# jiwoon-ahn/irn

Hardware: AMD Instinct MI355X
Metric: images/sec for CAM+random-walk label gen, VOC12 512^2 (random-walk label generation stage) (higher is better)
Workload: dtype f32

## Files before the change

irn_amd/csrc/affinity.hip:

```cpp
#include "path_unroll.hpp"

namespace irn {

namespace {

__device__ __forceinline__ float pow_beta(float a, float beta, int beta_int) {
    double b = (double)a;
    if (beta_int > 0) {
        double r = 1.0;
        int e = beta_int;
        while (e) {
            if (e & 1) r *= b;
            b *= b;
            e >>= 1;
        }
        return (float)r;
    }
    return (float)pow(b, (double)beta);
}

template <bool POW>
__global__ __launch_bounds__(256) void affinity_kernel(const AffJob *__restrict__ jobs,
                                                       const int *__restrict__ dir_start8,
                                                       const int *__restrict__ cell_off8, int n_dirs,
                                                       int radius, float beta, int beta_int) {
    extern __shared__ float tile[];
    const AffJob J = jobs[blockIdx.y];
    const int tiles_x = (J.sw + AFF_TW - 1) / AFF_TW;
    const int tiles_y = (J.sh + AFF_TH - 1) / AFF_TH;
    if ((int)blockIdx.x >= tiles_x * tiles_y) return;
    const int halo = radius - 1;
    const int LW = AFF_TW + 2 * halo;
    const int LH = AFF_TH + halo;
    const int ty0 = ((int)blockIdx.x / tiles_x) * AFF_TH;
    const int tx0 = ((int)blockIdx.x % tiles_x) * AFF_TW;

    for (int i = threadIdx.x; i < LH * LW; i += 256) {
        const int ly = i / LW, lx = i - ly * LW;
        const int gy = J.oy + ty0 + ly;
        const int gx = J.ox + tx0 + lx - halo;
        float v = 1.0f;
        if (gy < J.gh && gx >= 0 && gx < J.gw) v = J.edge[(long)gy * J.gw + gx];
        tile[i] = v;
    }
    __syncthreads();

    const int ly = threadIdx.x / AFF_TW, lx = threadIdx.x % AFF_TW;
    const int sy = ty0 + ly, sx = tx0 + lx;
    const bool valid = sy < J.sh && sx < J.sw;
    const int base = ly * LW + lx + halo;
    float *out = J.out + (long)sy * J.sw + sx;

    const float *tb = tile + base;
    for (int d = 0; d < n_dirs; ++d) {
        const int k0 = dir_start8[d], k1 = dir_start8[d + 1];
        float m0 = -INFINITY, m1 = -INFINITY;
        for (int k = k0; k < k1; k += 8) {
            const int4 oa = *reinterpret_cast<const int4 *>(cell_off8 + k);
            const int4 ob = *reinterpret_cast<const int4 *>(cell_off8 + k + 4);
            const float a0 = tb[oa.x], a1 = tb[oa.y], a2 = tb[oa.z], a3 = tb[oa.w];
            const float b0 = tb[ob.x], b1 = tb[ob.y], b2 = tb[ob.z], b3 = tb[ob.w];
            m0 = max3(max3(m0, a0, a1), a2, a3);
            m1 = max3(max3(m1, b0, b1), b2, b3);
        }
        const float m = max3(m0, m1, m1);
        float a = 1.0f - m;
        if (POW) a = pow_beta(a, beta, beta_int);
        if (valid) out[(long)d * J.plane_stride] = a;
    }
}

template <int R>
__global__ __launch_bounds__(256) void affinity_unrolled_kernel(const AffJob *__restrict__ jobs, int beta_int) {
    constexpr int HALO = R - 1, LW = AFF_TW + 2 * HALO, LH = AFF_TH + HALO, ND = kPaths<R>.n_dirs;
    __shared__ float tile[LH * LW];
    const AffJob J = jobs[blockIdx.y];
    const int tiles_x = (J.sw + AFF_TW - 1) / AFF_TW;
    const int tiles_y = (J.sh + AFF_TH - 1) / AFF_TH;
    if ((int)blockIdx.x >= tiles_x * tiles_y) return;
    const int ty0 = ((int)blockIdx.x / tiles_x) * AFF_TH;
    const int tx0 = ((int)blockIdx.x % tiles_x) * AFF_TW;
    for (int i = threadIdx.x; i < LH * LW; i += 256) {
        const int ly = i / LW, lx = i - ly * LW;
        const int gy = J.oy + ty0 + ly;
        const int gx = J.ox + tx0 + lx - HALO;
        float v = 1.0f;
        if (gy < J.gh && gx >= 0 && gx < J.gw) v = J.edge[(long)gy * J.gw + gx];
        tile[i] = v;
    }
    __syncthreads();
    const int ly = threadIdx.x / AFF_TW, lx = threadIdx.x % AFF_TW;
    const int sy = ty0 + ly, sx = tx0 + lx;
    const bool valid = sy < J.sh && sx < J.sw;
    const float *tb = tile + ly * LW + lx;
    float *out = J.out + (long)sy * J.sw + sx;
    static_for<ND>([&](auto id) __attribute__((always_inline)) {
        constexpr int d = decltype(id)::value;
        double b = (double)(1.0f - path_max<R, d>(tb)), r = 1.0;
        for (int e = beta_int; e; e >>= 1) {
            if (e & 1) r *= b;
            b *= b;
        }
        if (valid) *out = (float)r;
        out += J.plane_stride;
    });
}

__global__ __launch_bounds__(256) void affinity_backward_kernel(const AffJob *__restrict__ jobs,
                                                                const float *const *__restrict__ grad_aff,
                                                                float *const *__restrict__ grad_edge,
                                                                const int *__restrict__ dir_start,
                                                                const int *__restrict__ cell_dy,
                                                                const int *__restrict__ cell_dx, int n_dirs, int radius) {
    extern __shared__ float tile[];
    const AffJob J = jobs[blockIdx.y];
    const int tiles_x = (J.sw + AFF_TW - 1) / AFF_TW;
    const int tiles_y = (J.sh + AFF_TH - 1) / AFF_TH;
    if ((int)blockIdx.x >= tiles_x * tiles_y) return;
    const int halo = radius - 1;
    const int LW = AFF_TW + 2 * halo;
    const int LH = AFF_TH + halo;
    float *gtile = tile + LH * LW;
    const int ty0 = ((int)blockIdx.x / tiles_x) * AFF_TH;
    const int tx0 = ((int)blockIdx.x % tiles_x) * AFF_TW;
    for (int i = threadIdx.x; i < LH * LW; i += 256) {
        const int ly = i / LW, lx = i - ly * LW;
        const int gy = J.oy + ty0 + ly;
        const int gx = J.ox + tx0 + lx - halo;
        float v = 1.0f;
        if (gy < J.gh && gx >= 0 && gx < J.gw) v = J.edge[(long)gy * J.gw + gx];
        tile[i] = v;
        gtile[i] = 0.f;
    }
    __syncthreads();
    const int ly = threadIdx.x / AFF_TW, lx = threadIdx.x % AFF_TW;
    const int sy = ty0 + ly, sx = tx0 + lx;
    const bool valid = sy < J.sh && sx < J.sw;
    const int base = ly * LW + lx + halo;
    const float *ga = grad_aff[blockIdx.y] + (long)sy * J.sw + sx;
    if (valid) {
        for (int d = 0; d < n_dirs; ++d) {
            const int k0 = dir_start[d], k1 = dir_start[d + 1];
            float m = -INFINITY;
            int arg = 0;
            for (int k = k0; k < k1; ++k) {
                const int off = cell_dy[k] * LW + cell_dx[k];
                const float v = tile[base + off];
                if (v > m) {
                    m = v;
                    arg = off;
                }
            }
            atomicAdd(&gtile[base + arg], -ga[(long)d * J.plane_stride]);
        }
    }
    __syncthreads();
    float *ge = grad_edge[blockIdx.y];
    for (int i = threadIdx.x; i < LH * LW; i += 256) {
        const float g = gtile[i];
        if (g == 0.f) continue;
        const int py = i / LW, px = i - py * LW;
        const int gy = J.oy + ty0 + py;
        const int gx = J.ox + tx0 + px - halo;
        if (gy < J.gh && gx >= 0 && gx < J.gw) unsafeAtomicAdd(ge + (long)gy * J.gw + gx, g);
    }
}

}

int launch_affinity(const AffJob *jobs_dev, int n_jobs, int max_sh, int max_sw, const DeviceTable &tab,
                    bool with_pow, float beta, hipStream_t stream) {
    const int tiles = cdiv(max_sh, AFF_TH) * cdiv(max_sw, AFF_TW);
    const int halo = tab.radius - 1;
    const size_t lds = sizeof(float) * (AFF_TH + halo) * (AFF_TW + 2 * halo);
    dim3 grid(tiles, n_jobs);
    int beta_int = 0;
    if (with_pow && beta == (float)(int)beta && beta >= 1.0f && beta <= 64.0f) beta_int = (int)beta;
    if (with_pow && beta_int > 0 && tab.order == 1 && tab.radius == 10)
        hipLaunchKernelGGL(affinity_unrolled_kernel<10>, grid, dim3(256), 0, stream, jobs_dev, beta_int);
    else if (with_pow && beta_int > 0 && tab.order == 1 && tab.radius == 5)
        hipLaunchKernelGGL(affinity_unrolled_kernel<5>, grid, dim3(256), 0, stream, jobs_dev, beta_int);
    else if (with_pow)
        hipLaunchKernelGGL(affinity_kernel<true>, grid, dim3(256), lds, stream, jobs_dev, tab.dir_start8,
                           tab.cell_off8, tab.n_dirs, tab.radius, beta, beta_int);
    else
        hipLaunchKernelGGL(affinity_kernel<false>, grid, dim3(256), lds, stream, jobs_dev, tab.dir_start8,
                           tab.cell_off8, tab.n_dirs, tab.radius, beta, beta_int);
    IRN_LAUNCH_CHECK("affinity_kernel");
    return IRN_OK;
}

}

using namespace irn;

extern "C" int irn_version(void) { return 100; }

extern "C" const char *irn_last_error(void) { return last_error_slot().c_str(); }

extern "C" int irn_path_count(int radius, int *n_dirs, int *n_cells) {
    if (radius < 2 || radius > IRN_MAX_RADIUS || !n_dirs || !n_cells)
        return fail(IRN_ERR_ARG, "irn_path_count: radius must be in [2,%d]", IRN_MAX_RADIUS);
    PathTable t = build_path_table(radius, 0);
    *n_dirs = t.n_dirs();
    *n_cells = t.n_cells();
    return IRN_OK;
}

extern "C" int irn_path_table(int radius, int order, int32_t *dst_dydx, int32_t *path_start,
                              int32_t *cells_dydx) {
    if (radius < 2 || radius > IRN_MAX_RADIUS || (order != 0 && order != 1) || !dst_dydx || !path_start ||
        !cells_dydx)
        return fail(IRN_ERR_ARG, "irn_path_table: bad argument");
    PathTable t = build_path_table(radius, order);
    for (int i = 0; i < t.n_dirs(); ++i) {
        dst_dydx[2 * i] = t.dy[i];
        dst_dydx[2 * i + 1] = t.dx[i];
    }
    for (int i = 0; i <= t.n_dirs(); ++i) path_start[i] = t.start[i];
    for (int i = 0; i < t.n_cells(); ++i) {
        cells_dydx[2 * i] = t.cy[i];
        cells_dydx[2 * i + 1] = t.cx[i];
    }
    return IRN_OK;
}

extern "C" int irn_edge_to_affinity(const float *edge_dev, int batch, int hp, int wp, int radius,
                                    float *aff_dev, void *stream_) {
    hipStream_t stream = (hipStream_t)stream_;
    if (!edge_dev || !aff_dev || batch < 1 || radius < 2 || radius > IRN_MAX_RADIUS)
        return fail(IRN_ERR_ARG, "irn_edge_to_affinity: bad argument");
    const int rf = radius - 1;
    const int sh = hp - rf, sw = wp - 2 * rf;
    if (sh < 1 || sw < 1)
        return fail(IRN_ERR_ARG, "irn_edge_to_affinity: grid %dx%d too small for radius %d", hp, wp, radius);
    const DeviceTable *tab = nullptr;
    int rc = get_device_table(radius, 0, &tab);
    if (rc) return rc;
    std::vector<AffJob> jobs(batch);
    const long ns = (long)sh * sw;
    for (int b = 0; b < batch; ++b) {
        AffJob &j = jobs[b];
        j.edge = edge_dev + (long)b * hp * wp;
        j.out = aff_dev + (long)b * tab->n_dirs * ns;
        j.gh = hp; j.gw = wp; j.oy = 0; j.ox = rf; j.sh = sh; j.sw = sw;
        j.plane_stride = ns;
    }
    AffJob *jobs_dev = nullptr;
    rc = scratch_upload(jobs.data(), sizeof(AffJob) * batch, (void **)&jobs_dev, stream);
    if (rc) return rc;
    rc = launch_affinity(jobs_dev, batch, sh, sw, *tab, false, 0.f, stream);
    if (rc) return rc;
    return scratch_release(stream);
}

extern "C" int irn_edge_to_affinity_backward(const float *edge_dev, const float *grad_aff_dev, int batch, int hp, int wp,
                                             int radius, float *grad_edge_dev, void *stream_) {
    hipStream_t stream = (hipStream_t)stream_;
    if (!edge_dev || !grad_aff_dev || !grad_edge_dev || batch < 1 || radius < 2 || radius > IRN_MAX_RADIUS)
        return fail(IRN_ERR_ARG, "irn_edge_to_affinity_backward: bad argument");
    const int rf = radius - 1;
    const int sh = hp - rf, sw = wp - 2 * rf;
    if (sh < 1 || sw < 1)
        return fail(IRN_ERR_ARG, "irn_edge_to_affinity_backward: grid %dx%d too small for radius %d", hp, wp, radius);
    const DeviceTable *tab = nullptr;
    int rc = get_device_table(radius, 0, &tab);
    if (rc) return rc;
    const long ns = (long)sh * sw;
    std::vector<char> host(sizeof(AffJob) * batch + 2 * sizeof(void *) * batch);
    AffJob *jobs = (AffJob *)host.data();
    const float **gas = (const float **)(host.data() + sizeof(AffJob) * batch);
    float **ges = (float **)(host.data() + sizeof(AffJob) * batch + sizeof(void *) * batch);
    for (int b = 0; b < batch; ++b) {
        AffJob &j = jobs[b];
        j.edge = edge_dev + (long)b * hp * wp;
        j.out = nullptr;
        j.gh = hp; j.gw = wp; j.oy = 0; j.ox = rf; j.sh = sh; j.sw = sw;
        j.plane_stride = ns;
        gas[b] = grad_aff_dev + (long)b * tab->n_dirs * ns;
        ges[b] = grad_edge_dev + (long)b * hp * wp;
    }
    char *dev = nullptr;
    rc = scratch_upload(host.data(), host.size(), (void **)&dev, stream);
    if (rc) return rc;
    IRN_HIP_TRY(hipMemsetAsync(grad_edge_dev, 0, sizeof(float) * (size_t)batch * hp * wp, stream));
    const int tiles = cdiv(sh, AFF_TH) * cdiv(sw, AFF_TW);
    const size_t lds = 2 * sizeof(float) * (AFF_TH + rf) * (AFF_TW + 2 * rf);
    hipLaunchKernelGGL(affinity_backward_kernel, dim3(tiles, batch), dim3(256), lds, stream, (const AffJob *)dev,
                       (const float *const *)(dev + sizeof(AffJob) * batch),
                       (float *const *)(dev + sizeof(AffJob) * batch + sizeof(void *) * batch), tab->dir_start, tab->cell_dy,
                       tab->cell_dx, tab->n_dirs, radius);
    IRN_LAUNCH_CHECK("affinity_backward_kernel");
    return scratch_release(stream);
}

namespace {
__global__ __launch_bounds__(256) void pair_disp_kernel(const float *__restrict__ disp, float *__restrict__ out, int hp,
                                                        int wp, int rf, int n_dirs, const int *__restrict__ dir_dy,
                                                        const int *__restrict__ dir_dx) {
    const int ch = hp - rf, cw = wp - 2 * rf;
    const int s = blockIdx.x * 256 + threadIdx.x;
    if (s >= ch * cw) return;
    const int y = s / cw, x = s - y * cw;
    const float *plane = disp + (size_t)blockIdx.y * hp * wp;
    float *o = out + (size_t)blockIdx.y * n_dirs * ch * cw + s;
    const float src = plane[y * wp + rf + x];
    for (int d = 0; d < n_dirs; ++d)
        o[(size_t)d * ch * cw] = src - plane[(y + dir_dy[d]) * wp + rf + x + dir_dx[d]];
}

__global__ __launch_bounds__(256) void pair_disp_backward_kernel(const float *__restrict__ gout, float *__restrict__ gdisp,
                                                                 int hp, int wp, int rf, int n_dirs,
                                                                 const int *__restrict__ dir_dy, const int *__restrict__ dir_dx) {
    const int ch = hp - rf, cw = wp - 2 * rf;
    const int p = blockIdx.x * 256 + threadIdx.x;
    if (p >= hp * wp) return;
    const int Y = p / wp, X = p - Y * wp;
    const float *g = gout + (size_t)blockIdx.y * n_dirs * ch * cw;
    const int xs = X - rf;
    float acc = 0.f;
    if (Y < ch && xs >= 0 && xs < cw)
        for (int d = 0; d < n_dirs; ++d) acc += g[(size_t)d * ch * cw + Y * cw + xs];
    for (int d = 0; d < n_dirs; ++d) {
        const int yy = Y - dir_dy[d], xx = xs - dir_dx[d];
        if (yy >= 0 && yy < ch && xx >= 0 && xx < cw) acc -= g[(size_t)d * ch * cw + yy * cw + xx];
    }
    gdisp[(size_t)blockIdx.y * hp * wp + p] = acc;
}

int pair_disp_args(const char *who, const void *a, const void *b, int batch, int channels, int hp, int wp, int radius,
                   const DeviceTable **tab) {
    if (!a || !b || batch < 1 || channels < 1 || radius < 2 || radius > IRN_MAX_RADIUS)
        return fail(IRN_ERR_ARG, "%s: bad argument", who);
    if (hp - (radius - 1) < 1 || wp - 2 * (radius - 1) < 1)
        return fail(IRN_ERR_ARG, "%s: grid %dx%d too small for radius %d", who, hp, wp, radius);
    if ((long)batch * channels > 65535) return fail(IRN_ERR_ARG, "%s: batch * channels must be <= 65535", who);
    return get_device_table(radius, 0, tab);
}
}

extern "C" int irn_pair_displacement(const float *disp_dev, int batch, int channels, int hp, int wp, int radius,
                                     float *out_dev, void *stream) {
    const DeviceTable *tab = nullptr;
    if (int rc = pair_disp_args("irn_pair_displacement", disp_dev, out_dev, batch, channels, hp, wp, radius, &tab)) return rc;
    const int rf = radius - 1;
    hipLaunchKernelGGL(pair_disp_kernel, dim3(cdiv((hp - rf) * (wp - 2 * rf), 256), batch * channels), dim3(256), 0,
                       (hipStream_t)stream, disp_dev, out_dev, hp, wp, rf, tab->n_dirs, tab->dir_dy, tab->dir_dx);
    IRN_LAUNCH_CHECK("pair_disp_kernel");
    return IRN_OK;
}

extern "C" int irn_pair_displacement_backward(const float *grad_out_dev, int batch, int channels, int hp, int wp,
                                              int radius, float *grad_disp_dev, void *stream) {
    const DeviceTable *tab = nullptr;
    if (int rc = pair_disp_args("irn_pair_displacement_backward", grad_out_dev, grad_disp_dev, batch, channels, hp, wp,
                                radius, &tab))
        return rc;
    hipLaunchKernelGGL(pair_disp_backward_kernel, dim3(cdiv(hp * wp, 256), batch * channels), dim3(256), 0,
                       (hipStream_t)stream, grad_out_dev, grad_disp_dev, hp, wp, radius - 1, tab->n_dirs, tab->dir_dy,
                       tab->dir_dx);
    IRN_LAUNCH_CHECK("pair_disp_backward_kernel");
    return IRN_OK;
}
```

irn_amd/csrc/kernels.hpp:

```cpp
#pragma once
#include "common.hpp"

namespace irn {

struct DeviceTable {
    int radius = 0, order = 0, n_dirs = 0, n_cells = 0;
    int *dir_dy = nullptr, *dir_dx = nullptr;
    int *dir_start = nullptr;
    int *cell_dy = nullptr, *cell_dx = nullptr;
    int *cell_off8 = nullptr;
    int *dir_start8 = nullptr;
    int *plane_tab = nullptr;
    PathTable host;
};

int get_device_table(int radius, int order, const DeviceTable **out);

int scratch_upload(const void *host, size_t bytes, void **dev_out, hipStream_t stream);
int scratch_release(hipStream_t stream);

constexpr int kAffTileH = 8, kAffTileW = 32;

struct AffJob {
    const float *edge;
    float *out;
    int gh, gw;
    int oy, ox;
    int sh, sw;
    long plane_stride;
};

int launch_affinity(const AffJob *jobs_dev, int n_jobs, int max_sh, int max_sw, const DeviceTable &tab,
                    bool with_pow, float beta, hipStream_t stream);

}
```

irn_amd/csrc/path_unroll.hpp:

```cpp
#pragma once
#include <utility>

#include "kernels.hpp"

namespace irn {

constexpr int AFF_TH = kAffTileH;
constexpr int AFF_TW = kAffTileW;

__device__ __forceinline__ float max3(float a, float b, float c) {
    float r;
    asm("v_max3_f32 %0, %1, %2, %3" : "=v"(r) : "v"(a), "v"(b), "v"(c));
    return r;
}

template <int R>
struct Paths {
    static constexpr int kMaxDirs = 2 * R * R, kMaxCells = 32 * R * R;
    int n_dirs = 0, n_cells = 0;
    signed char dy[kMaxDirs] = {}, dx[kMaxDirs] = {};
    short start[kMaxDirs + 1] = {};
    signed char cy[kMaxCells] = {}, cx[kMaxCells] = {};
    constexpr void add(int y, int x) {
        dy[n_dirs] = (signed char)y;
        dx[n_dirs] = (signed char)x;
        const int lsq = y * y + x * x;
        const int x_lo = x < 0 ? x : 0, x_hi = x < 0 ? 0 : x;
        for (int py = 0; py <= y; ++py)
            for (int px = x_lo; px <= x_hi; ++px) {
                const int cross = y * px - x * py;
                if (cross * cross < lsq) {
                    cy[n_cells] = (signed char)py;
                    cx[n_cells] = (signed char)px;
                    ++n_cells;
                }
            }
        start[++n_dirs] = (short)n_cells;
    }
    constexpr Paths() {
        for (int x = 1; x < R; ++x) add(0, x);
        for (int y = 1; y < R; ++y)
            for (int x = -R + 1; x < R; ++x)
                if (x * x + y * y < R * R) add(y, x);
    }
};
template <int R>
inline constexpr Paths<R> kPaths{};

template <int... Is, typename F>
__device__ __forceinline__ void static_for_impl(std::integer_sequence<int, Is...>, F &&f) {
    (f(std::integral_constant<int, Is>{}), ...);
}
template <int N, typename F>
__device__ __forceinline__ void static_for(F &&f) {
    static_for_impl(std::make_integer_sequence<int, N>{}, f);
}

template <int R, int D>
__device__ __forceinline__ float path_max(const float *tb) {
    constexpr int LW = AFF_TW + 2 * (R - 1), HALO = R - 1;
    constexpr int k0 = kPaths<R>.start[D], n = kPaths<R>.start[D + 1] - k0;
    constexpr auto off = [](int k) constexpr { return kPaths<R>.cy[k] * LW + kPaths<R>.cx[k] + HALO; };
    float m = tb[off(k0)];
    static_for<(n - 1) / 2>([&](auto ik) __attribute__((always_inline)) {
        constexpr int k = k0 + 1 + 2 * decltype(ik)::value;
        m = max3(m, tb[off(k)], tb[off(k + 1)]);
    });
    if constexpr ((n - 1) % 2 == 1) {
        const float v = tb[off(k0 + n - 1)];
        m = max3(m, v, v);
    }
    return m;
}

}
```

irn_amd/csrc/walk.hip:

```cpp
#include <algorithm>
#include <cmath>
#include <mutex>

#include "walk_ctx.hpp"

namespace irn {


namespace {


__global__ __launch_bounds__(256) void zero_pad_kernel(const WalkImg *__restrict__ imgs, int n_dirs) {
    const WalkImg I = imgs[blockIdx.y];
    const int d = blockIdx.x;
    if (d >= n_dirs) return;
    float *plane = I.wts + (long)d * I.plane_stride;
    for (int i = threadIdx.x; i < I.front_pad; i += 256) plane[-1 - i] = 0.f;
    const long n = (long)I.h * I.w;
    const long end = I.plane_stride - I.front_pad;
    for (long i = n + threadIdx.x; i < end; i += 256) plane[i] = 0.f;
}

__global__ __launch_bounds__(256) void degree_kernel(const WalkImg *__restrict__ imgs,
                                                     const int *__restrict__ dir_dy,
// ... 454 lines not shown
    } else {
        return fail(IRN_ERR_ARG, "irn_walk_set_option: unknown option '%s'", name);
    }
    ctx->n = 0;
    return IRN_OK;
}

extern "C" int irn_walk_enable_timing(irn_walk_ctx *ctx, int enable) {
    if (!ctx) return fail(IRN_ERR_ARG, "null ctx");
    ctx->timing = enable ? 1 : 0;
    return IRN_OK;
}

extern "C" int irn_walk_last_sweep_ms(irn_walk_ctx *ctx, float *ms, int *n_launches) {
    if (!ctx || !ms || !n_launches) return fail(IRN_ERR_ARG, "null argument");
    if (ctx->ev_used == 0) return fail(IRN_ERR_STATE, "no timed run recorded");
    float total = 0.f;
    for (size_t i = 0; i + 1 < ctx->ev_used; i += 2) {
        float t = 0.f;
        IRN_HIP_TRY(hipEventSynchronize(ctx->ev_pool[i + 1]));
        IRN_HIP_TRY(hipEventElapsedTime(&t, ctx->ev_pool[i], ctx->ev_pool[i + 1]));
        total += t;
    }
    *ms = total;
    *n_launches = ctx->pending_launches;
    ctx->ev_used = 0;
    ctx->pending_launches = 0;
    return IRN_OK;
}

extern "C" int irn_walk_configure(irn_walk_ctx *ctx, int n_images, const int32_t *h, const int32_t *w,
                                  const int32_t *c, size_t *workspace_bytes) {
    if (!ctx || !h || !w || !c || !workspace_bytes || n_images < 1)
        return fail(IRN_ERR_ARG, "irn_walk_configure: bad argument");
    const int R = ctx->radius;
    if (ctx->run_done_ev && ctx->last_valid) IRN_HIP_TRY(hipEventSynchronize(ctx->run_done_ev));
    ctx->last_valid = false;
    ctx->n = 0;
    ctx->h.assign(h, h + n_images);
    ctx->w.assign(w, w + n_images);
    ctx->c.assign(c, c + n_images);
    ctx->off_wts.resize(n_images);
    ctx->off_deg.resize(n_images);
    ctx->off_xa.resize(n_images);
    ctx->off_xb.resize(n_images);
    ctx->off_xc.resize(n_images);
    ctx->plane_stride.resize(n_images);
    ctx->front_pad.resize(n_images);
    size_t off = 0;
    ctx->max_h = ctx->max_w = ctx->max_n = 0;
    bool blocked_ok = ctx->variant >= 1;
    for (int i = 0; i < n_images; ++i) {
        if (h[i] < 1 || w[i] < 1 || c[i] < 1 || c[i] > 0xffff)
            return fail(IRN_ERR_ARG, "irn_walk_configure: image %d has invalid size %dx%d c=%d", i, h[i], w[i], c[i]);
        const size_t npx = (size_t)h[i] * w[i];
        const int fp = (int)round_up((size_t)(R - 1) * w[i] + (R - 1), 64);
        const long ps = (long)round_up(fp + npx + 8, 64);
        ctx->front_pad[i] = fp;
        ctx->plane_stride[i] = ps;
        ctx->off_wts[i] = off;
        off += round_up(sizeof(float) * ps * ctx->tab->n_dirs, 256);
        ctx->off_deg[i] = off;
        off += round_up(sizeof(double) * npx, 256);
        ctx->off_xa[i] = off;
        off += round_up(8 * npx * c[i] + 64, 256);
        ctx->off_xb[i] = off;
        off += round_up(8 * npx * c[i] + 64, 256);
        ctx->off_xc[i] = off;
        off += round_up(8 * npx * c[i] + 64, 256);
        ctx->max_h = std::max(ctx->max_h, (int)h[i]);
        ctx->max_w = std::max(ctx->max_w, (int)w[i]);
        ctx->max_n = std::max(ctx->max_n, (int)npx);
        if (w[i] < R) blocked_ok = false;
    }
    ctx->ws_bytes = off;
    ctx->all_blocked_ok = blocked_ok;

    std::vector<int4> map;
    for (int k = 0; k < 5; ++k) ctx->cls_begin[k] = ctx->cls_count[k] = 0;
    ctx->max_nch = 1;
    if (blocked_ok) {
        const int NX = 8;
        for (int cls = 4; cls >= 1; --cls) {
            while (map.size() % NX) map.push_back(make_int4(-1, 0, 0, 0));
            ctx->cls_begin[cls] = (int)map.size();
            std::vector<std::vector<int4>> q(NX);
            std::vector<size_t> load(NX, 0);
            for (int i = 0; i < n_images; ++i) {
                int best = 0;
                for (int k = 1; k < NX; ++k)
                    if (load[k] < load[best]) best = k;
                for (int c0 = 0; c0 < c[i]; c0 += kMaxChunk) {
                    const int nch = std::min(kMaxChunk, c[i] - c0);
                    if (nch != cls) continue;
                    ctx->max_nch = std::max(ctx->max_nch, nch);
                    for (int ty = 0; ty < h[i]; ty += kTileH)
                        for (int tx = 0; tx < w[i]; tx += kTileW) {
                            q[best].push_back(make_int4(i, ty, tx, c0 | (nch << 16)));
                            ++load[best];
                        }
                }
            }
            size_t depth = 0;
            for (auto &v : q) depth = std::max(depth, v.size());
            const size_t begin = map.size();
            for (size_t sl = 0; sl < depth; ++sl)
                for (int k = 0; k < NX; ++k) map.push_back(sl < q[k].size() ? q[k][sl] : make_int4(-1, 0, 0, 0));
            while (map.size() > begin && map.back().x < 0) map.pop_back();
            ctx->cls_count[cls] = (int)(map.size() - begin);
        }
    }
    ctx->map_len = (int)map.size();

    if (n_images > ctx->cap_imgs) {
        if (ctx->imgs_dev) (void)hipFree(ctx->imgs_dev);
        if (ctx->jobs_dev) (void)hipFree(ctx->jobs_dev);
        ctx->imgs_dev = nullptr;
        ctx->jobs_dev = nullptr;
        IRN_HIP_TRY(hipMalloc((void **)&ctx->imgs_dev, sizeof(WalkImg) * n_images));
        IRN_HIP_TRY(hipMalloc((void **)&ctx->jobs_dev, sizeof(AffJob) * n_images));
        ctx->cap_imgs = n_images;
    }
    const size_t stage_need = (sizeof(WalkImg) + sizeof(AffJob)) * (size_t)n_images;
    if (stage_need > ctx->stage_cap) {
        for (int k = 0; k < 2; ++k) {
            if (ctx->stage[k]) (void)hipHostFree(ctx->stage[k]);
            ctx->stage[k] = nullptr;
            IRN_HIP_TRY(hipHostMalloc(&ctx->stage[k], stage_need, hipHostMallocDefault));
            if (!ctx->stage_ev[k]) IRN_HIP_TRY(hipEventCreateWithFlags(&ctx->stage_ev[k], hipEventDisableTiming));
        }
        ctx->stage_cap = stage_need;
    }
    if ((int)map.size() > ctx->cap_map) {
        if (ctx->map_dev) (void)hipFree(ctx->map_dev);
        ctx->map_dev = nullptr;
        IRN_HIP_TRY(hipMalloc((void **)&ctx->map_dev, sizeof(int4) * map.size()));
        ctx->cap_map = (int)map.size();
    }
    if (!map.empty())
        IRN_HIP_TRY(hipMemcpy(ctx->map_dev, map.data(), sizeof(int4) * map.size(), hipMemcpyHostToDevice));
    if (ctx->variant == 2) {
        const int rc = resident_configure(ctx);
        if (rc) return rc;
    } else {
        ctx->res_ok = false;
    }
    ctx->n = n_images;
    *workspace_bytes = ctx->ws_bytes;
    return IRN_OK;
}

template <int R, int CH>
static int launch_blocked_cls(irn_walk_ctx *ctx, int phase, int last, int cheb, float ck, hipStream_t stream) {
    const int nb = ctx->cls_count[CH];
    if (nb <= 0) return IRN_OK;
    return launch_sweep<R, CH>(ctx->imgs_dev, ctx->map_dev + ctx->cls_begin[CH], ctx->tab->plane_tab, nb,
                               phase, last, cheb, ck, stream);
}

template <int R>
static int launch_blocked(irn_walk_ctx *ctx, int phase, int last, int cheb, float ck, hipStream_t const *st) {
    int rc = launch_blocked_cls<R, 1>(ctx, phase, last, cheb, ck, st[0]);
    if (!rc) rc = launch_blocked_cls<R, 2>(ctx, phase, last, cheb, ck, st[1]);
    if (!rc) rc = launch_blocked_cls<R, 3>(ctx, phase, last, cheb, ck, st[2]);
    if (!rc) rc = launch_blocked_cls<R, 4>(ctx, phase, last, cheb, ck, st[3]);
    return rc;
}

static int timing_events(irn_walk_ctx *ctx, hipEvent_t *ev0, hipEvent_t *ev1) {
    while (ctx->ev_pool.size() < ctx->ev_used + 2) {
        hipEvent_t e;
        IRN_HIP_TRY(hipEventCreate(&e));
        ctx->ev_pool.push_back(e);
    }
    *ev0 = ctx->ev_pool[ctx->ev_used];
    *ev1 = ctx->ev_pool[ctx->ev_used + 1];
    return IRN_OK;
}

int irn::streaming_run(irn_walk_ctx *ctx, int n_sweeps, hipStream_t stream, bool timed) {
    const DeviceTable &tab = *ctx->tab;
    const int n = ctx->n;
    const int pix_blocks = cdiv(ctx->max_n, 256);
    {
        const int rc_s = walk_schedule(ctx, n_sweeps, stream);
        if (rc_s) return rc_s;
    }
    const bool cheb = ctx->sched_cheb;
    const int n_steps = ctx->sched_steps;
    hipLaunchKernelGGL(degree_kernel, dim3(pix_blocks, n), dim3(256), 0, stream, ctx->imgs_dev, tab.dir_dy, tab.dir_dx,
                       tab.n_dirs);
    IRN_LAUNCH_CHECK("degree_kernel");
    ctx->deg_stale = false;
    hipLaunchKernelGGL(x0_kernel, dim3(pix_blocks, n), dim3(256), 0, stream, ctx->imgs_dev, n_sweeps == 0 ? 1 : 0,
                       cheb ? 1 : 0, cheb ? (float)ctx->sched_coef[0] : 0.f);
    IRN_LAUNCH_CHECK("x0_kernel");

    const bool blocked = ctx->variant >= 1 && ctx->all_blocked_ok;
    hipStream_t st[4] = {stream, stream, stream, stream};
    int n_side = 0;
    if (blocked && n_steps > 0) {
        int big = 1;
        for (int k = 2; k <= 4; ++k)
            if (ctx->cls_count[k] > ctx->cls_count[big]) big = k;
        for (int k = 1; k <= 4; ++k) {
            if (k == big || ctx->cls_count[k] == 0) continue;
            if (!ctx->side[n_side]) {
                IRN_HIP_TRY(hipStreamCreateWithFlags(&ctx->side[n_side], hipStreamNonBlocking));
                IRN_HIP_TRY(hipEventCreateWithFlags(&ctx->ev_join[n_side], hipEventDisableTiming));
            }
            st[k - 1] = ctx->side[n_side++];
        }
        if (n_side && !ctx->ev_fork) IRN_HIP_TRY(hipEventCreateWithFlags(&ctx->ev_fork, hipEventDisableTiming));
    }
    hipEvent_t ev0 = nullptr, ev1 = nullptr;
    int rc = IRN_OK;
    if (timed) {
        rc = timing_events(ctx, &ev0, &ev1);
        if (rc) return rc;
        IRN_HIP_TRY(hipEventRecord(ev0, stream));
    }
    if (n_side) {
        IRN_HIP_TRY(hipEventRecord(ctx->ev_fork, stream));
        for (int k = 0; k < n_side; ++k) IRN_HIP_TRY(hipStreamWaitEvent(ctx->side[k], ctx->ev_fork, 0));
    }
    for (int t = 0; t < n_steps; ++t) {
        const int last = (t == n_steps - 1) ? 1 : 0;
        const int mode = cheb ? (t == 0 ? 1 : 2) : 0;
        const float ck = cheb ? (float)ctx->sched_coef[t + 1] : 0.f;
        if (blocked) {
            rc = ctx->radius == 5 ? launch_blocked<5>(ctx, t, last, mode, ck, st) : launch_blocked<10>(ctx, t, last, mode, ck, st);
            if (rc) return rc;
        } else {
            hipLaunchKernelGGL(sweep_generic_kernel, dim3(pix_blocks, n), dim3(256), 0, stream, ctx->imgs_dev,
                               tab.dir_dy, tab.dir_dx, tab.n_dirs, t, last, mode, ck);
            IRN_LAUNCH_CHECK("sweep_generic_kernel");
        }
    }
    for (int k = 0; k < n_side; ++k) {
        IRN_HIP_TRY(hipEventRecord(ctx->ev_join[k], ctx->side[k]));
        IRN_HIP_TRY(hipStreamWaitEvent(stream, ctx->ev_join[k], 0));
    }
    if (timed) {
        IRN_HIP_TRY(hipEventRecord(ev1, stream));
        ctx->ev_used += 2;
        ctx->pending_launches += n_steps;
    }
    return IRN_OK;
}

extern "C" int irn_walk_run(irn_walk_ctx *ctx, const float *const *edge_dev, const float *const *cam_dev,
                            const int32_t *const *inst_map_dev, const int32_t *k_inst,
                            float *const *out_dev, float beta, int n_sweeps, void *workspace_dev,
                            size_t workspace_bytes, void *stream_) {
    hipStream_t stream = (hipStream_t)stream_;
    if (!ctx || !edge_dev || !cam_dev || !out_dev || !workspace_dev)
        return fail(IRN_ERR_ARG, "irn_walk_run: null argument");
    if (ctx->n < 1) return fail(IRN_ERR_STATE, "irn_walk_run: irn_walk_configure has not been called");
    if (workspace_bytes < ctx->ws_bytes)
        return fail(IRN_ERR_STATE, "irn_walk_run: workspace of %zu bytes, %zu needed", workspace_bytes, ctx->ws_bytes);
    if (!(beta > 0.f)) return fail(IRN_ERR_ARG, "irn_walk_run: beta must be > 0 (got %g)", (double)beta);
    if (n_sweeps < 0) return fail(IRN_ERR_ARG, "irn_walk_run: n_sweeps must be >= 0");
    if (((uintptr_t)workspace_dev & 255) != 0)
        return fail(IRN_ERR_ARG, "irn_walk_run: workspace must be 256-byte aligned");

    const int n = ctx->n;
    const int slot = ctx->stage_next;
    ctx->stage_next ^= 1;
    IRN_HIP_TRY(hipEventSynchronize(ctx->stage_ev[slot]));
    if (ctx->res_err_host && ctx->res_err_host[0] != 0) {
        const int rc_prev = irn_walk_check(ctx);
        if (rc_prev) return rc_prev;
    }
    WalkImg *imgs = (WalkImg *)ctx->stage[slot];
    AffJob *jobs = (AffJob *)(imgs + n);
    char *ws = (char *)workspace_dev;
    for (int i = 0; i < n; ++i) {
        if (!edge_dev[i] || !cam_dev[i] || !out_dev[i])
            return fail(IRN_ERR_ARG, "irn_walk_run: null pointer for image %d", i);
        WalkImg &I = imgs[i];
        I.edge = edge_dev[i];
        I.cam = cam_dev[i];
        I.inst = (inst_map_dev && inst_map_dev[i]) ? inst_map_dev[i] : nullptr;
        I.k_inst = (I.inst && k_inst) ? k_inst[i] : 1;
        if (I.inst && (I.k_inst < 1 || ctx->c[i] % I.k_inst != 0))
            return fail(IRN_ERR_ARG, "irn_walk_run: image %d: c=%d is not a multiple of k_inst=%d", i, ctx->c[i], I.k_inst);
        I.out = out_dev[i];
        I.wts = (float *)(ws + ctx->off_wts[i]) + ctx->front_pad[i];
        I.inv_deg = (double *)(ws + ctx->off_deg[i]);
        I.xa = (float *)(ws + ctx->off_xa[i]);
        I.xb = (float *)(ws + ctx->off_xb[i]);
        I.xc = (float *)(ws + ctx->off_xc[i]);
        I.h = ctx->h[i];
        I.w = ctx->w[i];
        I.C = ctx->c[i];
        I.plane_stride = ctx->plane_stride[i];
        I.front_pad = ctx->front_pad[i];
        I.n_dirs = ctx->tab->n_dirs;
        AffJob &J = jobs[i];
        J.edge = I.edge;
        J.out = I.wts;
        J.gh = I.h; J.gw = I.w; J.oy = 0; J.ox = 0; J.sh = I.h; J.sw = I.w;
        J.plane_stride = I.plane_stride;
    }
    IRN_HIP_TRY(hipMemcpyAsync(ctx->imgs_dev, imgs, sizeof(WalkImg) * n, hipMemcpyHostToDevice, stream));
    IRN_HIP_TRY(hipMemcpyAsync(ctx->jobs_dev, jobs, sizeof(AffJob) * n, hipMemcpyHostToDevice, stream));
    IRN_HIP_TRY(hipEventRecord(ctx->stage_ev[slot], stream));

    const DeviceTable &tab = *ctx->tab;
    hipLaunchKernelGGL(zero_pad_kernel, dim3(tab.n_dirs, n), dim3(256), 0, stream, ctx->imgs_dev, tab.n_dirs);
    IRN_LAUNCH_CHECK("zero_pad_kernel");
    int rc = launch_affinity(ctx->jobs_dev, n, ctx->max_h, ctx->max_w, tab, true, beta, stream);
    if (rc) return rc;
    const bool resident = ctx->variant == 2 && ctx->res_ok && n_sweeps > 0;
    ctx->deg_stale = resident;
    ctx->last_stream = stream;
    ctx->last_n_sweeps = n_sweeps;
    ctx->last_resident = resident;
    ctx->last_valid = true;
    hipEvent_t ev0 = nullptr, ev1 = nullptr;
    if (ctx->timing && resident) {
        rc = timing_events(ctx, &ev0, &ev1);
        if (rc) return rc;
        IRN_HIP_TRY(hipEventRecord(ev0, stream));
    }
    if (resident) {
        rc = resident_run(ctx, n_sweeps, stream);
        if (rc) return rc;
        if (ctx->timing) {
            IRN_HIP_TRY(hipEventRecord(ev1, stream));
            ctx->ev_used += 2;
            ctx->pending_launches += ctx->sched_steps;
        }
    } else {
        rc = streaming_run(ctx, n_sweeps, stream, ctx->timing != 0);
        if (rc) return rc;
    }
    if (!ctx->run_done_ev) IRN_HIP_TRY(hipEventCreateWithFlags(&ctx->run_done_ev, hipEventDisableTiming));
    IRN_HIP_TRY(hipEventRecord(ctx->run_done_ev, stream));
    return IRN_OK;
}

extern "C" int irn_walk_check(irn_walk_ctx *ctx) {
    if (!ctx) return fail(IRN_ERR_ARG, "null ctx");
    if (!ctx->res_err_host) return IRN_OK;
    if (ctx->res_err_host[0] != 0) {
        const unsigned img = ctx->res_err_host[1], t = ctx->res_err_host[2], wg = ctx->res_err_host[3];
        ctx->res_err_host[0] = 0;
        return fail(IRN_ERR_STATE, "resident walk timed out: workgroup %u waiting for state of sweep %u of image %u "
                                   "(a neighbouring tile never published it)", wg, t, img);
    }
    return IRN_OK;
}

extern "C" int irn_walk_sync(irn_walk_ctx *ctx, int *fell_back) {
    if (!ctx) return fail(IRN_ERR_ARG, "null ctx");
    if (fell_back) *fell_back = 0;
    if (!ctx->last_valid || !ctx->run_done_ev) return IRN_OK;
    IRN_HIP_TRY(hipEventSynchronize(ctx->run_done_ev));
    if (!ctx->last_resident || !ctx->res_err_host || ctx->res_err_host[0] == 0) return IRN_OK;
    ctx->res_err_host[0] = 0;
    ctx->last_resident = false;
    ++ctx->fallback_runs;
    if (fell_back) *fell_back = 1;
    int rc = streaming_run(ctx, ctx->last_n_sweeps, ctx->last_stream, false);
    if (rc) return rc;
    IRN_HIP_TRY(hipStreamSynchronize(ctx->last_stream));
    return IRN_OK;
}

extern "C" int irn_walk_fallback_runs(irn_walk_ctx *ctx) { return ctx ? ctx->fallback_runs : 0; }

extern "C" int irn_walk_tuning(irn_walk_ctx *ctx, int *poll_delay, int *placement, float *probe_ms4) {
    if (!ctx) return fail(IRN_ERR_ARG, "irn_walk_tuning: null ctx");
    if (poll_delay) *poll_delay = ctx->res_poll_delay;
    if (placement) *placement = ctx->res_placement;
    if (probe_ms4)
        for (int k = 0; k < 4; ++k) probe_ms4[k] = ctx->res_poll_probe_ms[k];
    return IRN_OK;
}

extern "C" int irn_walk_plan_rounds(int radius, int n_images, const int32_t *h, const int32_t *w, const int32_t *channels,
                                    int n_workgroups, int placement, int32_t *jobs_out, int cap_rounds, int *n_rounds) {
    if (!h || !w || !channels || !n_rounds || n_images < 1 || n_workgroups < 1 || cap_rounds < 0 || (cap_rounds > 0 && !jobs_out))
        return fail(IRN_ERR_ARG, "irn_walk_plan_rounds: bad argument");
    if (radius != 5 && radius != 10) return fail(IRN_ERR_ARG, "irn_walk_plan_rounds: the persistent walk exists for radius 5 and 10");
    std::vector<int> jobs;
    int nr = 0;
    if (!irn::resident_plan_rounds(radius, n_images, h, w, channels, n_workgroups, placement, jobs, &nr)) {
        *n_rounds = 0;
        return IRN_OK;
    }
    *n_rounds = nr;
    if (nr > cap_rounds) return cap_rounds == 0 ? IRN_OK : fail(IRN_ERR_ARG, "irn_walk_plan_rounds: jobs_out too small");
    std::copy(jobs.begin(), jobs.end(), jobs_out);
    return IRN_OK;
}

extern "C" int irn_walk_read_profile(irn_walk_ctx *ctx, long long *host_out) {
    if (!ctx || !host_out) return fail(IRN_ERR_ARG, "null argument");
    if (!ctx->res_prof_dev) return fail(IRN_ERR_STATE, "option 'profile' is off");
    IRN_HIP_TRY(hipMemcpy(host_out, ctx->res_prof_dev, 2 * 256 * 4 * sizeof(long long), hipMemcpyDeviceToHost));
    return IRN_OK;
}

extern "C" int irn_walk_export_weights(irn_walk_ctx *ctx, int image, float *w_dev, double *inv_deg_dev,
                                       void *workspace_dev, void *stream_) {
    hipStream_t stream = (hipStream_t)stream_;
    if (!ctx || ctx->n < 1 || image < 0 || image >= ctx->n || !workspace_dev)
        return fail(IRN_ERR_ARG, "irn_walk_export_weights: bad argument");
    char *ws = (char *)workspace_dev;
    const size_t npx = (size_t)ctx->h[image] * ctx->w[image];
    if (w_dev) {
        const float *src = (const float *)(ws + ctx->off_wts[image]) + ctx->front_pad[image];
        IRN_HIP_TRY(hipMemcpy2DAsync(w_dev, sizeof(float) * npx, src, sizeof(float) * ctx->plane_stride[image],
                                     sizeof(float) * npx, ctx->tab->n_dirs, hipMemcpyDeviceToDevice, stream));
    }
    if (inv_deg_dev && ctx->deg_stale) {
        hipLaunchKernelGGL(degree_kernel, dim3(cdiv(ctx->max_n, 256), ctx->n), dim3(256), 0, stream, ctx->imgs_dev,
                           ctx->tab->dir_dy, ctx->tab->dir_dx, ctx->tab->n_dirs);
        IRN_LAUNCH_CHECK("degree_kernel");
        ctx->deg_stale = false;
    }
    if (inv_deg_dev)
        IRN_HIP_TRY(hipMemcpyAsync(inv_deg_dev, ws + ctx->off_deg[image], sizeof(double) * npx,
                                   hipMemcpyDeviceToDevice, stream));
    return IRN_OK;
}
```

Baseline: 19410.

## Compute two pixels per lane in affinity kernel with wide LDS reads, fuse pad zeroing

Replaces the unrolled affinity kernel with a wide variant. Each lane handles two adjacent pixels, reading from two shifted LDS copies of the tile with batched inline-asm ds_read_b64, and writes vectorised float2 outputs when aligned. The tile grows to 16 rows and the row stride is padded to avoid bank conflicts. Extra blocks in the same grid zero the plane pads, removing the separate zero_pad kernel launch. The cost is more LDS per block and more register pressure, plus fragile inline asm that waits on each read batch.

Measured after the change: 19670, median of 6. 1.3% higher.

```diff
diff --git a/irn_amd/csrc/affinity.hip b/irn_amd/csrc/affinity.hip
--- a/irn_amd/csrc/affinity.hip
+++ b/irn_amd/csrc/affinity.hip
@@ -70,40 +70,85 @@
     }
 }
 
-template <int R>
-__global__ __launch_bounds__(256) void affinity_unrolled_kernel(const AffJob *__restrict__ jobs, int beta_int) {
-    constexpr int HALO = R - 1, LW = AFF_TW + 2 * HALO, LH = AFF_TH + HALO, ND = kPaths<R>.n_dirs;
-    __shared__ float tile[LH * LW];
+constexpr int AFF_P = 2;
+constexpr int AFF_PAD_BLOCKS = 8;
+
+typedef __attribute__((address_space(1))) float global_float;
+template <int P>
+using global_floatP = __attribute__((address_space(1))) floatP<P>;
+
+template <int R, int P>
+__global__ __launch_bounds__(256) void affinity_wide_kernel(const AffJob *__restrict__ jobs, int beta_int, int max_tiles) {
+    using T = WideTile<R, P>;
+    constexpr int ND = kPaths<R>.n_dirs;
+    __shared__ __attribute__((aligned(16))) float tile[P * T::COPY];
     const AffJob J = jobs[blockIdx.y];
-    const int tiles_x = (J.sw + AFF_TW - 1) / AFF_TW;
-    const int tiles_y = (J.sh + AFF_TH - 1) / AFF_TH;
+    if ((int)blockIdx.x >= max_tiles) {
+        const long n = (long)J.sh * J.sw;
+        for (int d = (int)blockIdx.x - max_tiles; d < ND; d += AFF_PAD_BLOCKS) {
+            float *plane = J.out + (long)d * J.plane_stride;
+            for (int i = threadIdx.x; i < J.pad_front; i += 256) plane[i - J.pad_front] = 0.f;
+            for (int i = threadIdx.x; i < J.pad_tail; i += 256) plane[n + i] = 0.f;
+        }
+        return;
+    }
+    const int tiles_x = (J.sw + T::TW - 1) / T::TW;
+    const int tiles_y = (J.sh + T::TH - 1) / T::TH;
     if ((int)blockIdx.x >= tiles_x * tiles_y) return;
-    const int ty0 = ((int)blockIdx.x / tiles_x) * AFF_TH;
-    const int tx0 = ((int)blockIdx.x % tiles_x) * AFF_TW;
-    for (int i = threadIdx.x; i < LH * LW; i += 256) {
-        const int ly = i / LW, lx = i - ly * LW;
+    const int ty0 = ((int)blockIdx.x / tiles_x) * T::TH;
+    const int tx0 = ((int)blockIdx.x % tiles_x) * T::TW;
+    for (int i = threadIdx.x; i < T::LH * T::LW; i += 256) {
+        const int ly = i / T::LW, lx = i - ly * T::LW;
         const int gy = J.oy + ty0 + ly;
-        const int gx = J.ox + tx0 + lx - HALO;
+        const int gx = J.ox + tx0 + lx - T::HALO;
         float v = 1.0f;
         if (gy < J.gh && gx >= 0 && gx < J.gw) v = J.edge[(long)gy * J.gw + gx];
-        tile[i] = v;
+#pragma unroll
+        for (int s = 0; s < P; ++s)
+            if (lx >= s) tile[s * T::COPY + ly * T::STRIDE + lx - s] = v;
     }
     __syncthreads();
-    const int ly = threadIdx.x / AFF_TW, lx = threadIdx.x % AFF_TW;
+    const int ly = threadIdx.x / T::LANES_X, lx = (threadIdx.x % T::LANES_X) * P;
     const int sy = ty0 + ly, sx = tx0 + lx;
-    const bool valid = sy < J.sh && sx < J.sw;
-    const float *tb = tile + ly * LW + lx;
-    float *out = J.out + (long)sy * J.sw + sx;
-    static_for<ND>([&](auto id) __attribute__((always_inline)) {
-        constexpr int d = decltype(id)::value;
-        double b = (double)(1.0f - path_max<R, d>(tb)), r = 1.0;
-        for (int e = beta_int; e; e >>= 1) {
-            if (e & 1) r *= b;
-            b *= b;
-        }
-        if (valid) *out = (float)r;
-        out += J.plane_stride;
-    });
+    const unsigned tb = (unsigned)(uintptr_t)(__attribute__((address_space(3))) float *)tile + 4 * (ly * T::STRIDE + lx);
+    global_float *out = (global_float *)J.out + (long)sy * J.sw + sx;
+    const int n_valid = sy < J.sh ? min(P, J.sw - sx) : 0;
+    const bool vec = n_valid == P && ((uintptr_t)out & (4 * P - 1)) == 0 && J.plane_stride % P == 0;
+    auto planes = [&](auto wide) __attribute__((always_inline)) {
+        static_for<ND>([&](auto id) __attribute__((always_inline)) {
+            constexpr int d = decltype(id)::value;
+            const floatP<P> m = path_max_wide<R, P, d>(tb);
+            double b[P], r[P];
+            static_for<P>([&](auto ip) __attribute__((always_inline)) { b[decltype(ip)::value] = (double)(1.0f - m[decltype(ip)::value]); });
+            int e = beta_int;
+            for (; e > 1 && !(e & 1); e >>= 1)
+                static_for<P>([&](auto ip) __attribute__((always_inline)) { b[decltype(ip)::value] *= b[decltype(ip)::value]; });
+            static_for<P>([&](auto ip) __attribute__((always_inline)) { r[decltype(ip)::value] = b[decltype(ip)::value]; });
+            for (e >>= 1; e; e >>= 1) {
+                static_for<P>([&](auto ip) __attribute__((always_inline)) { b[decltype(ip)::value] *= b[decltype(ip)::value]; });
+                if (e & 1) {
+                    asm volatile("");
+                    static_for<P>([&](auto ip) __attribute__((always_inline)) { r[decltype(ip)::value] *= b[decltype(ip)::value]; });
+                }
+            }
+            floatP<P> w;
+            static_for<P>([&](auto ip) __attribute__((always_inline)) { w[decltype(ip)::value] = (float)r[decltype(ip)::value]; });
+            if constexpr (decltype(wide)::value) {
+                *reinterpret_cast<global_floatP<P> *>(out) = w;
+            } else {
+                static_for<P>([&](auto ip) __attribute__((always_inline)) {
+                    constexpr int p = decltype(ip)::value;
+                    if (p < n_valid) out[p] = w[p];
+                });
+            }
+            out += J.plane_stride;
+        });
+    };
+    if (__builtin_amdgcn_ballot_w64(n_valid > 0 && !vec) == 0) {
+        if (vec) planes(std::true_type{});
+    } else {
+        planes(std::false_type{});
+    }
 }
 
 __global__ __launch_bounds__(256) void affinity_backward_kernel(const AffJob *__restrict__ jobs,
@@ -168,19 +213,31 @@
 
 }
 
+bool affinity_writes_pads(const DeviceTable &tab, bool with_pow, float beta) {
+    return with_pow && tab.order == 1 && (tab.radius == 10 || tab.radius == 5) && beta == (float)(int)beta &&
+           beta >= 1.0f && beta <= 64.0f;
+}
+
 int launch_affinity(const AffJob *jobs_dev, int n_jobs, int max_sh, int max_sw, const DeviceTable &tab,
                     bool with_pow, float beta, hipStream_t stream) {
-    const int tiles = cdiv(max_sh, AFF_TH) * cdiv(max_sw, AFF_TW);
     const int halo = tab.radius - 1;
     const size_t lds = sizeof(float) * (AFF_TH + halo) * (AFF_TW + 2 * halo);
-    dim3 grid(tiles, n_jobs);
     int beta_int = 0;
     if (with_pow && beta == (float)(int)beta && beta >= 1.0f && beta <= 64.0f) beta_int = (int)beta;
-    if (with_pow && beta_int > 0 && tab.order == 1 && tab.radius == 10)
-        hipLaunchKernelGGL(affinity_unrolled_kernel<10>, grid, dim3(256), 0, stream, jobs_dev, beta_int);
-    else if (with_pow && beta_int > 0 && tab.order == 1 && tab.radius == 5)
-        hipLaunchKernelGGL(affinity_unrolled_kernel<5>, grid, dim3(256), 0, stream, jobs_dev, beta_int);
-    else if (with_pow)
+    if (affinity_writes_pads(tab, with_pow, beta)) {
+        using T = WideTile<10, AFF_P>;
+        static_assert(T::TW == WideTile<5, AFF_P>::TW && T::TH == WideTile<5, AFF_P>::TH, "one tile for both radii");
+        const int tiles = cdiv(max_sh, T::TH) * cdiv(max_sw, T::TW);
+        dim3 grid(tiles + AFF_PAD_BLOCKS, n_jobs);
+        if (tab.radius == 10)
+            hipLaunchKernelGGL((affinity_wide_kernel<10, AFF_P>), grid, dim3(256), 0, stream, jobs_dev, beta_int, tiles);
+        else
+            hipLaunchKernelGGL((affinity_wide_kernel<5, AFF_P>), grid, dim3(256), 0, stream, jobs_dev, beta_int, tiles);
+        IRN_LAUNCH_CHECK("affinity_wide_kernel");
+        return IRN_OK;
+    }
+    dim3 grid(cdiv(max_sh, AFF_TH) * cdiv(max_sw, AFF_TW), n_jobs);
+    if (with_pow)
         hipLaunchKernelGGL(affinity_kernel<true>, grid, dim3(256), lds, stream, jobs_dev, tab.dir_start8,
                            tab.cell_off8, tab.n_dirs, tab.radius, beta, beta_int);
     else
diff --git a/irn_amd/csrc/kernels.hpp b/irn_amd/csrc/kernels.hpp
--- a/irn_amd/csrc/kernels.hpp
+++ b/irn_amd/csrc/kernels.hpp
@@ -28,9 +28,12 @@
     int oy, ox;
     int sh, sw;
     long plane_stride;
+    int pad_front;
+    int pad_tail;
 };
 
 int launch_affinity(const AffJob *jobs_dev, int n_jobs, int max_sh, int max_sw, const DeviceTable &tab,
                     bool with_pow, float beta, hipStream_t stream);
+bool affinity_writes_pads(const DeviceTable &tab, bool with_pow, float beta);
 
 }
diff --git a/irn_amd/csrc/path_unroll.hpp b/irn_amd/csrc/path_unroll.hpp
--- a/irn_amd/csrc/path_unroll.hpp
+++ b/irn_amd/csrc/path_unroll.hpp
@@ -73,4 +73,88 @@
     return m;
 }
 
+template <int R, int P>
+struct WideTile {
+    static_assert(P == 2, "8-byte LDS reads");
+    static constexpr int TW = 32, TH = 16;
+    static constexpr int LANES_X = TW / P, HALO = R - 1, LW = TW + 2 * HALO, LH = TH + HALO;
+    static constexpr int STRIDE = (LW + 31) / 64 * 64 + 32;
+    static constexpr int COPY = LH * STRIDE;
+    static_assert(TW % P == 0 && LANES_X * TH == 256, "one lane per P pixels, 256 lanes");
+    static_assert(STRIDE >= LW && STRIDE % P == 0 && COPY % P == 0, "aligned rows and copies");
+    static_assert(STRIDE % 64 == 32 && LANES_X * P == 32, "two rows of a ds_read_b64 group on disjoint banks");
+    static_assert(P * COPY * 4 <= 65536, "LDS offsets are 16-bit immediates");
+};
+
+template <int P>
+using floatP = float __attribute__((ext_vector_type(P)));
+
+#define IRN_DS_RD(i) IRN_DS_OP " %" #i ", %[a] offset:%[o" #i "]\n\t"
+#define IRN_DS_READS(P_)                                                                                               \
+    template <int O0, int O1, int O2, int O3, int O4, int O5, int O6, int O7>                                          \
+    __device__ __forceinline__ void lds_read8(unsigned a, floatP<P_> *v) {                                             \
+        asm volatile(IRN_DS_RD(0) IRN_DS_RD(1) IRN_DS_RD(2) IRN_DS_RD(3) IRN_DS_RD(4) IRN_DS_RD(5) IRN_DS_RD(6)        \
+                     IRN_DS_RD(7) "s_waitcnt lgkmcnt(0)"                                                               \
+                     : "=&v"(v[0]), "=&v"(v[1]), "=&v"(v[2]), "=&v"(v[3]), "=&v"(v[4]), "=&v"(v[5]), "=&v"(v[6]),      \
+                       "=&v"(v[7])                                                                                     \
+                     : [a] "v"(a), [o0] "n"(O0), [o1] "n"(O1), [o2] "n"(O2), [o3] "n"(O3), [o4] "n"(O4), [o5] "n"(O5), \
+                       [o6] "n"(O6), [o7] "n"(O7));                                                                    \
+    }                                                                                                                  \
+    template <int O0, int O1, int O2, int O3>                                                                          \
+    __device__ __forceinline__ void lds_read4(unsigned a, floatP<P_> *v) {                                             \
+        asm volatile(IRN_DS_RD(0) IRN_DS_RD(1) IRN_DS_RD(2) IRN_DS_RD(3) "s_waitcnt lgkmcnt(0)"                        \
+                     : "=&v"(v[0]), "=&v"(v[1]), "=&v"(v[2]), "=&v"(v[3])                                              \
+                     : [a] "v"(a), [o0] "n"(O0), [o1] "n"(O1), [o2] "n"(O2), [o3] "n"(O3));                            \
+    }                                                                                                                  \
+    template <int O0, int O1>                                                                                          \
+    __device__ __forceinline__ void lds_read2(unsigned a, floatP<P_> *v) {                                             \
+        asm volatile(IRN_DS_RD(0) IRN_DS_RD(1) "s_waitcnt lgkmcnt(0)"                                                  \
+                     : "=&v"(v[0]), "=&v"(v[1])                                                                        \
+                     : [a] "v"(a), [o0] "n"(O0), [o1] "n"(O1));                                                        \
+    }                                                                                                                  \
+    template <int O0>                                                                                                  \
+    __device__ __forceinline__ void lds_read1(unsigned a, floatP<P_> *v) {                                             \
+        asm volatile(IRN_DS_RD(0) "s_waitcnt lgkmcnt(0)" : "=&v"(v[0]) : [a] "v"(a), [o0] "n"(O0));                    \
+    }
+#define IRN_DS_OP "ds_read_b64"
+IRN_DS_READS(2)
+#undef IRN_DS_OP
+#undef IRN_DS_READS
+#undef IRN_DS_RD
+
+template <int R, int P, int D>
+__device__ __forceinline__ floatP<P> path_max_wide(unsigned a) {
+    using T = WideTile<R, P>;
+    constexpr int k0 = kPaths<R>.start[D], n = kPaths<R>.start[D + 1] - k0;
+    constexpr auto off = [](int i) constexpr {
+        const int c = kPaths<R>.cx[k0 + i] + T::HALO, s = c % P;
+        return 4 * (s * T::COPY + kPaths<R>.cy[k0 + i] * T::STRIDE + c - s);
+    };
+    floatP<P> v[n];
+    static_for<n / 8>([&](auto ib) __attribute__((always_inline)) {
+        constexpr int i = 8 * decltype(ib)::value;
+        lds_read8<off(i), off(i + 1), off(i + 2), off(i + 3), off(i + 4), off(i + 5), off(i + 6), off(i + 7)>(a, v + i);
+    });
+    constexpr int i4 = n / 8 * 8, i2 = i4 + (n & 4), i1 = i2 + (n & 2);
+    if constexpr (n & 4) lds_read4<off(i4), off(i4 + 1), off(i4 + 2), off(i4 + 3)>(a, v + i4);
+    if constexpr (n & 2) lds_read2<off(i2), off(i2 + 1)>(a, v + i2);
+    if constexpr (n & 1) lds_read1<off(i1)>(a, v + i1);
+    static_assert(off(0) % (4 * P) == 0 && off(n - 1) % (4 * P) == 0 && off(n - 1) + 4 * P <= 4 * P * T::COPY, "aligned, inside");
+    floatP<P> m = v[0];
+    static_for<(n - 1) / 2>([&](auto ik) __attribute__((always_inline)) {
+        constexpr int k = 1 + 2 * decltype(ik)::value;
+        static_for<P>([&](auto ip) __attribute__((always_inline)) {
+            constexpr int p = decltype(ip)::value;
+            m[p] = max3(m[p], v[k][p], v[k + 1][p]);
+        });
+    });
+    if constexpr ((n - 1) % 2 == 1) {
+        static_for<P>([&](auto ip) __attribute__((always_inline)) {
+            constexpr int p = decltype(ip)::value;
+            m[p] = max3(m[p], v[n - 1][p], v[n - 1][p]);
+        });
+    }
+    return m;
 }
+
+}
diff --git a/irn_amd/csrc/walk.hip b/irn_amd/csrc/walk.hip
--- a/irn_amd/csrc/walk.hip
+++ b/irn_amd/csrc/walk.hip
@@ -780,14 +780,18 @@
         J.out = I.wts;
         J.gh = I.h; J.gw = I.w; J.oy = 0; J.ox = 0; J.sh = I.h; J.sw = I.w;
         J.plane_stride = I.plane_stride;
+        J.pad_front = I.front_pad;
+        J.pad_tail = (int)(I.plane_stride - I.front_pad - (long)I.h * I.w);
     }
     IRN_HIP_TRY(hipMemcpyAsync(ctx->imgs_dev, imgs, sizeof(WalkImg) * n, hipMemcpyHostToDevice, stream));
     IRN_HIP_TRY(hipMemcpyAsync(ctx->jobs_dev, jobs, sizeof(AffJob) * n, hipMemcpyHostToDevice, stream));
     IRN_HIP_TRY(hipEventRecord(ctx->stage_ev[slot], stream));
 
     const DeviceTable &tab = *ctx->tab;
-    hipLaunchKernelGGL(zero_pad_kernel, dim3(tab.n_dirs, n), dim3(256), 0, stream, ctx->imgs_dev, tab.n_dirs);
-    IRN_LAUNCH_CHECK("zero_pad_kernel");
+    if (!affinity_writes_pads(tab, true, beta)) {
+        hipLaunchKernelGGL(zero_pad_kernel, dim3(tab.n_dirs, n), dim3(256), 0, stream, ctx->imgs_dev, tab.n_dirs);
+        IRN_LAUNCH_CHECK("zero_pad_kernel");
+    }
     int rc = launch_affinity(ctx->jobs_dev, n, ctx->max_h, ctx->max_w, tab, true, beta, stream);
     if (rc) return rc;
     const bool resident = ctx->variant == 2 && ctx->res_ok && n_sweeps > 0;
```
